# AI-ON/Few-Shot-Music-Generation

Hardware: AMD Instinct MI355X
Metric: episodes/s (LSTM-baseline train step, synthetic vocab=10k seq_len=128 5-way/5-shot h=512) (higher is better)
Workload: dtype f32 (bf16x3-split products, fp32 accumulate)

## Files before the change

### few-shot-music-generation_amd/csrc/api_debug.hip

```cpp
#include "fsmg_model.h"

using namespace fsmg;
using namespace fsmg_host;


extern "C" {

int fsmg_debug_clock_begin(fsmg_handle h, int32_t microseconds) {
    if (!h || microseconds <= 0 || microseconds > 1000000) return FSMG_ERR_INVALID;
    BEGIN_CALL(h, true);
    if (!h->probe) HIPCK(h, hipStreamCreateWithFlags(&h->probe, hipStreamNonBlocking));
    if (!h->d_probe) HIPCK(h, hipMalloc((void**)&h->d_probe, 64));
    HIPCK(h, hipMemsetAsync(h->d_probe, 0, 64, h->probe));
    HIPCK(h, launch_clock_probe(h->probe, (long long)microseconds * 100, h->d_probe));
    return FSMG_OK;
}
int fsmg_debug_clock_end(fsmg_handle h, float* ghz) {
    if (!h || !ghz) return FSMG_ERR_INVALID;
    if (!h->probe || !h->d_probe) return fail(h, FSMG_ERR_STATE, "fsmg_debug_clock_end without fsmg_debug_clock_begin");
    BEGIN_CALL(h, true);
    unsigned long long v[2] = {0, 0};
    HIPCK(h, hipStreamSynchronize(h->probe));
    HIPCK(h, hipMemcpy(v, h->d_probe, sizeof(v), hipMemcpyDeviceToHost));
    *ghz = v[1] ? (float)((double)v[0] / (double)v[1] * 0.1) : 0.0f;
    return FSMG_OK;
}

int fsmg_debug_dims(fsmg_handle h, int32_t dims[5]) {
    if (!h || !dims) return FSMG_ERR_INVALID;
    dims[0] = h->Ep; dims[1] = h->Hp; dims[2] = h->V1p; dims[3] = h->lastB; dims[4] = h->T;
    return FSMG_OK;
}

int fsmg_debug_read(fsmg_handle h, const char* what, float* host, int64_t count) {
    if (!h || !what || !host || count <= 0) return FSMG_ERR_INVALID;
    BEGIN_CALL(h);
    const int64_t B = h->lastB, T = h->T, Hp = h->Hp, G4 = h->G4, rows = T * B;
    const float* src = nullptr; int64_t cap = 0;
    auto layer_of = [&](const char* prefix) -> int {
        const size_t n = std::strlen(prefix);
        if (std::strncmp(what, prefix, n) != 0) return -1;
        const int l = std::atoi(what + n);
        return (l >= 0 && l < h->L && std::strlen(what) > n) ? l : -1;
    };
    int l;
    if (!std::strcmp(what, "aux_tries")) { host[0] = (float)h->aux_tries; return FSMG_OK; }
    if (!std::strcmp(what, "fused_softmax")) { host[0] = h->fused_softmax ? 1.0f : 0.0f; if (count > 1) host[1] = h->fs_call ? 1.0f : 0.0f; return FSMG_OK; }
    if (!std::strcmp(what, "xcd_bx3")) { host[0] = h->xcd_bx3 ? 1.0f : 0.0f; return FSMG_OK; }
    if (!std::strcmp(what, "gemm_kinds")) {
        for (int64_t i = 0; i < count && i < 4; ++i) host[i] = (float)h->gemm_kinds[i];
        return FSMG_OK;
    }
    if (!std::strcmp(what, "xov_selfcheck")) {
        const float v[3] = {(float)h->xov_selfcheck_runs, (float)h->xov_passes, (float)h->xov_selfcheck_every};
        for (int64_t i = 0; i < count && i < 3; ++i) host[i] = v[i];
        return FSMG_OK;
    }
    if (!std::strcmp(what, "xcd_partitioned")) {
        host[0] = h->xov ? 1.0f : 0.0f;
        if (count > 1) { const int b = h->lastB > 0 ? h->lastB : 45, rpx = lstm_xcd16_packed_rows(b, h->Hp); host[1] = (h->xov && rpx > 0) ? (float)xov_first_free(b, h->Hp) : 8.0f; }
        if (count > 2) host[2] = h->xov_last ? 1.0f : 0.0f;
        return FSMG_OK;
    }
    if (!std::strcmp(what, "logits")) { src = h->logits; cap = rows * h->V1p; }
    else if (!std::strcmp(what, "dlogits")) { src = dlogits_buf(h); cap = rows * h->V1p; }
    else if (!std::strcmp(what, "lse")) { src = h->lse; cap = rows; }
    else if (!std::strcmp(what, "ce")) { src = h->ce; cap = rows; }
    else if (!std::strcmp(what, "row_weight")) { src = h->roww; cap = h->last_mask_groups > 0 ? rows : 0; }
    else if (!std::strcmp(what, "n_valid")) {
        if (count > h->last_mask_groups) return fail(h, FSMG_ERR_SIZE, "debug read larger than the buffer");
        std::vector<int> nv((size_t)count);
        HIPCK(h, hipStreamSynchronize(h->stream));
        HIPCK(h, hipMemcpy(nv.data(), h->d_nvalid, sizeof(int) * count, hipMemcpyDeviceToHost));
        for (int64_t i = 0; i < count; ++i) host[i] = (float)nv[(size_t)i];
        return FSMG_OK;
    }
    else if (!std::strcmp(what, "dx")) { src = h->dXemb; cap = rows * h->Ep; }
    else if (!std::strcmp(what, "dh")) { src = h->dH; cap = rows * Hp; }
    else if (!std::strcmp(what, "gnorm")) { src = h->d_gnorm; cap = 1; }
    else if (!std::strcmp(what, "tail")) { src = h->G + h->n_flat; cap = FSMG_GRAD_TAIL; }
    else if ((l = layer_of("gates")) >= 0) { src = h->Z[l]; cap = rows * G4; }
    else if ((l = layer_of("h")) >= 0) { src = h->Hs[l]; cap = (T + 1) * B * Hp; }
    else if ((l = layer_of("c")) >= 0) { src = h->Cs[l]; cap = (T + 1) * B * Hp; }
    else return fail(h, FSMG_ERR_NAME, std::string("unknown debug buffer '") + what + "'");
    if (count > cap) return fail(h, FSMG_ERR_SIZE, "debug read larger than the buffer");
    HIPCK(h, hipStreamSynchronize(h->stream));
    HIPCK(h, hipMemcpy(host, src, sizeof(float) * count, hipMemcpyDeviceToHost));
    return FSMG_OK;
}

int fsmg_debug_step_profile(fsmg_handle h, int32_t which, uint64_t* stamps, int64_t cap, int32_t* n_blocks,
                            int32_t* n_waves) {
    if (!h || !stamps || !n_blocks || !n_waves || h->lastB <= 0 || h->T < 3) return FSMG_ERR_INVALID;
    BEGIN_CALL(h);
    { const int rc_cs = ensure_cs(h); if (rc_cs != FSMG_OK) return rc_cs; }
    const int B = h->lastB, Hp = h->Hp, G4 = h->G4, l = h->L - 1, t = h->T / 2;
    const int nb = which == 0 ? (G4 / 16) * ((B + 15) / 16) : (Hp / 16) * ((B + 15) / 16);
    const int nw = which == 0 ? 4 : 8;
    const int64_t n = (int64_t)nb * nw * 8;
    if (cap < n) return fail(h, FSMG_ERR_SIZE, "stamp buffer too small");
    unsigned long long* d = nullptr;
    HIPCK(h, hipMalloc((void**)&d, sizeof(unsigned long long) * n));
    HIPCK(h, hipMemsetAsync(d, 0, sizeof(unsigned long long) * n, h->stream));
    for (int rep = 0; rep < 3; ++rep) {
        if (which == 0) {
            LstmFwdArgs a{};
            const size_t Bp16 = (size_t)(B + 15) / 16 * 16;
            a.KhF = h->khf + (size_t)(2 * l) * Hp * G4; a.hF_prev = h->HF[l] + (size_t)t * Bp16 * Hp;
// ... 54 lines not shown
```

### few-shot-music-generation_amd/csrc/api_schedule.hip

```cpp
#include "fsmg_model.h"

using namespace fsmg;
using namespace fsmg_host;

namespace fsmg_host {

bool use_ws_gemm(fsmg_model* h, int amode, int bmode, const GemmArgs& g, const Lane& ln) {
    const int mode = h->gemm_ws;
    if (!h->bx3 || mode == 0 || ln.lds_pad != 0 || g.xcd_first != 0) return false;
    if (mode == 2) return true;
    const int64_t tiles = ((g.M + 127) / 128) * (int64_t)((g.N + 127) / 128);
    if (amode == OP_KC && bmode == OP_XC) return g.K >= 384 && g.K <= 640 && tiles >= 512;
    if (amode == OP_XC && bmode == OP_XC) return tiles >= 256 && g.M <= 512;
    return g.K <= 4096;
}

bool use_h_gemm(fsmg_model* h, int amode, int bmode, const GemmArgs& g, const Lane& ln) {
    const int mode = h->gemm_h;
    if (!h->bx3 || mode == 0 || ln.lds_pad != 0 || g.xcd_first != 0) return false;
    if (amode == OP_XC && g.gather != nullptr && g.m_split == 0) return false;
    if (mode == 2) return true;
    const int64_t tiles = ((g.M + 255) / 256) * (int64_t)((g.N + 255) / 256);
    if (amode == OP_KC && bmode == OP_KC) return g.K >= 4096 && tiles >= 32;
    if (amode == OP_XC && bmode == OP_XC) {
// ... 37 lines not shown
        return FSMG_OK;
    }
    if (!deferred && slabs == h->slabs && h->slabs_owner != nullptr) GEMMCK(h->slabs_owner->flush());
    if (!deferred && slabs == h->slabs && h->side_pending) {
        HIPCK(h, hipStreamWaitEvent(h->stream, h->ev_side, 0));
        h->side_pending = false;
    }
    if (deferred && sq != nullptr && g.row_scale != nullptr) return fail(h, FSMG_ERR_STATE, "internal: row-scaled GEMM with squared-norm partials");
    float* C = g.C; float* colsum = g.colsum;
    g.C = slabs; g.c_slab = mn; g.ksplit = S;
    if (colsum) { g.colsum = cslabs; g.colsum_slab = g.N; }
    HIPCK(h, launch_gemm(h, s, amode, bmode, g, ln.lds_pad));
    if (deferred) {
        if (sq != nullptr && g.row_scale != nullptr) return fail(h, FSMG_ERR_STATE, "internal: row-scaled GEMM with squared-norm partials");
        GEMMCK(defer->room(colsum ? 2 : 1));
        GEMMCK(defer->reduce(slabs, mn, S, C, mn, sq, g.row_scale, g.N));
        if (colsum) GEMMCK(defer->reduce(cslabs, g.N, S, colsum, g.N));
        if (sq_done) *sq_done = sq != nullptr;
        return FSMG_OK;
    }
    HIPCK(h, launch_reduce_slabs2(s, slabs, mn, S, C, mn, cslabs, g.N, colsum, colsum ? g.N : 0));
    if (g.row_scale != nullptr) HIPCK(h, launch_scale_rows(s, C, g.row_scale, g.M, g.N));
    return FSMG_OK;
}

int select_xcd_format(fsmg_model* h, int B) {
    if (h->Hp != 1024 || !h->bx3 || h->xcd_bx3_forced || h->khx == nullptr || !(h->persist && h->xcd)) return FSMG_OK;
    const bool want = lstm_xcd_bx3_pays(B, (int)h->Hp) && B <= h->xcd_max_rows;
    if (want == h->xcd_bx3) return FSMG_OK;
    h->xcd_bx3 = want;
    drop_graphs(h);
    return repack_recurrent_weights(h, h->stream);
}

void choose_schedule(fsmg_model* h, int B, bool train) {
    h->ov_call = h->overlap && (h->overlap_forced || !use_xcd(h, B));
    h->xov_call = false;
    h->eager_call = h->eager && !h->ov_call && h->persist &&
                    (use_xcd(h, B) || lstm_fwd_chain_supported(B, h->Hp) || lstm_fwd_chain_rt_supported(B, h->Hp));
    if (train && h->xov && ((h->Hp == 512 && h->L == 1) || h->Hp == 1024) && h->xcd_bx3 && h->bx3 && !h->ov_call && h->aux != nullptr && use_xcd(h, B) &&
        (!h->timing || h->timing_only == "lstm_fwd" || h->timing_only == "lstm_bwd")) {
        const int rpx = lstm_xcd16_packed_rows(B, h->Hp);
        h->xov_call = rpx > 0 && xov_first_free(B, h->Hp) <= (h->Hp == 1024 ? 6 : 5);
        if (h->xov_call) h->eager_call = true;
    }
}
void xov_gate(fsmg_model* h, GemmArgs& g, int B) {
    const int rpx = lstm_xcd16_packed_rows(B, h->Hp);
    g.gate = h->xov_prog; g.gate_expect = lstm_xcd_active_blocks(B, rpx, h->Hp); g.gate_rows = B; g.gate_last = h->T - 1;
    g.gate_err = h->d_err; g.gate_spin = h->chain_spin_limit > 0 ? 200000 : 0; g.gate_every = h->xov_pub;
}
int gemm_restricted(fsmg_model* h, hipStream_t s, int amode, int bmode, GemmArgs g, int first, int* ctl) {
    g.bx3 = 3; g.xcd_first = first; g.work = ctl; g.stop = ctl + 2; g.claim = ctl + 4; g.work_limit = gemm_items(g);
    HIPCK(h, launch_gemm(h, s, amode, bmode, g, 0));
    return FSMG_OK;
}
int gemm_prepare_queue(fsmg_model* h, GemmArgs& g, int split, OpBatch* defer, bool* ok) {
    *ok = false;
    const int S = std::max(1, std::min(std::min(split, MAX_SPLIT), g.K / 256));
    const int64_t mn = (int64_t)g.M * g.N;
    const int64_t need = round_up((int64_t)S * mn, 64) + (g.colsum ? round_up((int64_t)S * g.N, 64) : 0);
    if (S < 2 || defer == nullptr || h->arena == nullptr || g.ldc != g.N || h->arena_off + need > h->arena_cap || g.row_scale != nullptr) return FSMG_OK;
    float* slabs = h->arena + h->arena_off; float* cslabs = slabs + round_up((int64_t)S * mn, 64);
    h->arena_off += need;
    float* C = g.C; float* colsum = g.colsum;
    g.C = slabs; g.c_slab = mn; g.ksplit = S; g.bx3 = 3;
    if (colsum) { g.colsum = cslabs; g.colsum_slab = g.N; }
    if (!xov_fits(g)) { h->arena_off -= need; g.C = C; g.colsum = colsum; g.ksplit = 1; return FSMG_OK; }
    GEMMCK(defer->room(colsum ? 2 : 1));
    GEMMCK(defer->reduce(slabs, mn, S, C, mn));
    if (colsum) GEMMCK(defer->reduce(cslabs, g.N, S, colsum, g.N));
    *ok = true;
    return FSMG_OK;
}
int gemm_cleanup(fsmg_model* h, hipStream_t s, int amode, int bmode, GemmArgs g, int* ctl) {
    g.bx3 = 3; g.xcd_first = -1; g.work = ctl; g.claim = ctl + 4;
    HIPCK(h, launch_gemm(h, s, amode, bmode, g, 0));
    return FSMG_OK;
}

}
```

### few-shot-music-generation_amd/csrc/fsmg_model.h

```cpp
#pragma once
#include <atomic>
#include <hip/hip_runtime.h>
#include <dlfcn.h>

#include <algorithm>
#include <cmath>
#include <cstdlib>
#include <new>
#include <cstdio>
#include <cstring>
#include <functional>
#include <map>
#include <mutex>
#include <string>
#include <vector>

#include "../../include/fsmg.h"
#include "fsmg_kernels.h"

namespace fsmg_host {
using namespace fsmg;
struct OpBatch;

inline int64_t round_up(int64_t x, int64_t m) { return (x + m - 1) / m * m; }
// ... 117 lines not shown
    float* inboxX = nullptr; int64_t inboxx_floats = 0;
    int* d_inbox_dirty = nullptr;
    int* tickets = nullptr;
    static constexpr int TICKET_LAUNCHES = 64;
    int ticket_next = 0;
    int64_t n_timeouts = 0, n_persist_launches = 0, n_xcd_launches = 0, n_step_launches = 0;
    bool khf_dirty = true;
    bool lazy_cs = true;
    bool cs_stale = false;
    float* slabs = nullptr;
    float* arena = nullptr;
    int64_t arena_cap = 0, arena_off = 0;
    bool warned_split = false;
    int* tok_first = nullptr; int* tok_count = nullptr;
    bool tok_table_open = false;
    bool last_bwd_xcd = false;
    bool eager = true, eager_call = false;
    const int* cur_sup = nullptr; const int* cur_qry = nullptr;
    float* colsum_slabs = nullptr;
    float* slabs2 = nullptr;
    float* colsum_slabs2 = nullptr;
    hipStream_t probe = nullptr;
    unsigned long long* d_probe = nullptr;
    hipStream_t aux = nullptr;
    int aux_tries = 0;
    static constexpr int NCHUNK = 16;
    static constexpr int nchunk = 8;
    static constexpr int nchunk_persist = 4;
    static constexpr int aux_blocks_persist = 2;
    static constexpr int aux_blocks_per_cu = 2;
    hipEvent_t ev_chunk[NCHUNK] = {};
    hipEvent_t ev_fork = nullptr, ev_join = nullptr;
    bool merge_dk = true;
    hipEvent_t ev_bucket[2] = {};
    bool overlap = true;
    bool overlap_forced = false;
    bool ov_call = false;
    int bx3 = 1;
    int gemm_h = 1;
    int gemm_ws = 1;
    int max_split = fsmg_host::MAX_SPLIT;
    long long gemm_kinds[4] = {};
    bool xov = false, xov_call = false;
    bool xov_eligible = false;
    bool bucket0_recorded = false;
    static constexpr int xov_dw_split = 4;
    static constexpr int xov_pub = 6;
    int xov_strikes = 0;
    bool xov_last = false;
    int xov_parts = 3;
    int* xov_prog = nullptr;
    static constexpr int XOV_CTL = 8192;
    int* xov_ctl = nullptr;
    int64_t slab_cap = 0;
    std::map<std::string, hipGraphExec_t> graphs;
    struct LaunchCounts { int64_t xcd = 0, persist = 0, step = 0; bool bwd_xcd = false; };
    std::map<std::string, LaunchCounts> graph_counts;
    char* gen = nullptr;
    size_t gen_bytes = 0;
    std::vector<fsmg_dstate_s*> dstates;
    std::vector<fsmg_cache_s*> caches;
    char* cat = nullptr;
    size_t cat_bytes = 0;

    void* comm = nullptr; bool own_comm = false; int world = 1, rank = 0;
    hipStream_t comm_stream = nullptr;
    hipEvent_t ev_comm = nullptr;
    int lastB = 0;
    bool have_grads = false;
    bool upd_split = false;
    bool upd_pending = false;
    hipEvent_t ev_upd_fork = nullptr, ev_upd = nullptr;
    float* d_decided = nullptr;
    fsmg_host::OpBatch* slabs_owner = nullptr;
    int xov_selfcheck_left = 2;
    int xov_selfcheck_every = 1000;
    long long xov_passes = 0, xov_selfcheck_runs = 0;
    bool xov_selfcheck_fault = false;
    long long seen_selfcheck_mismatch = 0;
    bool inplace_dlogits = true;
    bool fused_softmax = true;
    bool fs_call = false;
    float* Hsc = nullptr;
    float* crow = nullptr;
    long long seen_softmax_range = 0;
    bool tail_aside = true;
    bool side_pending = false;
    hipEvent_t ev_side_fork = nullptr, ev_side = nullptr;
    hipEvent_t ev_turn = nullptr, ev_turn_aux = nullptr;
    std::atomic<bool> capturing{false};
    std::string err;
    bool timing = false;
    std::string timing_only;
    std::map<std::string, fsmg_host::TimerClass> timers;
};

namespace fsmg_host {

extern thread_local std::string g_create_error;

inline int fail(fsmg_model* h, int code, const std::string& msg) {
    if (h) h->err = msg; else g_create_error = msg;
    return code;
}

template <class Config>
// ... 288 lines not shown
```

### few-shot-music-generation_amd/csrc/gemm.hip

```cpp
#include "fsmg_kernels.h"
#include "gemm_edge.h"
#include <cstdlib>
#include <algorithm>
#include <type_traits>

namespace fsmg {

typedef float f32x16 __attribute__((ext_vector_type(16)));

namespace {

#ifndef FSMG_GEMM_BK
#define FSMG_GEMM_BK 16
#endif
#ifndef FSMG_GEMM_BM
#define FSMG_GEMM_BM 128
#endif
constexpr int BM = FSMG_GEMM_BM, BN = 128, BK = FSMG_GEMM_BK;
constexpr int NTHREADS = 2 * BM;
constexpr int NWAVES = NTHREADS / 64;
constexpr int KQ = BK / 4;
template <int XW> struct Nld { static constexpr int v = XW * BK / 4 / NTHREADS; };
template <int MODE, int XW> struct TileLd { static constexpr int v = (MODE == OP_KC) ? XW + 1 : XW + 4; };

// ... 597 lines not shown
            }
#pragma unroll
            for (int i = 0; i < 2; ++i) {
                const float4 q = *reinterpret_cast<const float4*>(p[i]);
                v[4 * i] = q.x; v[4 * i + 1] = q.y; v[4 * i + 2] = q.z; v[4 * i + 3] = q.w;
                p[i] += step;
            }
        }
    }
    __device__ __forceinline__ void fetch_partial(int k0, int kend, int tid) {
        const long long adv = use_buf ? (long long)(so >> 2) : 0;
        so += sstep;
        if (MODE == OP_XC) {
            const int kh = tid / XW;
            if (gp != nullptr) {
#pragma unroll
                for (int i = 0; i < 8; ++i) v[i] = (k0 + 8 * kh + i < kend) ? p[0][(long long)gi[i] * ld_] : 0.0f;
                advance_ids();
                return;
            }
            const float* q = use_buf ? src_ + (vo[0] >> 2) + adv : p[0];
#pragma unroll
            for (int i = 0; i < 8; ++i) v[i] = (k0 + 8 * kh + i < kend) ? q[i * ld_] : 0.0f;
            if (!use_buf) p[0] += step;
        } else {
            const int kq = tid & 3;
#pragma unroll
            for (int i = 0; i < 2; ++i) {
                const float* q = use_buf ? src_ + (vo[i] >> 2) + adv : p[i];
#pragma unroll
                for (int e = 0; e < 4; ++e) v[4 * i + e] = (k0 + 4 * kq + e < kend) ? q[e] : 0.0f;
                if (!use_buf) p[i] += step;
            }
        }
    }
    __device__ __forceinline__ void load() {}
    __device__ __forceinline__ float sum8() const { return ((v[0] + v[1]) + (v[2] + v[3])) + ((v[4] + v[5]) + (v[6] + v[7])); }
    __device__ __forceinline__ void commit(unsigned char* tile) const {
        unsigned w[3][4];
        split8(v, w);
#pragma unroll
        for (int pl = 0; pl < 3; ++pl) {
            if (MODE == OP_XC) {
                *reinterpret_cast<uint4*>(tile + pl * PLANE + lds_ofs[0]) = make_uint4(w[pl][0], w[pl][1], w[pl][2], w[pl][3]);
            } else {
                *reinterpret_cast<uint2*>(tile + pl * PLANE + lds_ofs[0]) = make_uint2(w[pl][0], w[pl][1]);
                *reinterpret_cast<uint2*>(tile + pl * PLANE + lds_ofs[1]) = make_uint2(w[pl][2], w[pl][3]);
            }
        }
    }
};

typedef __attribute__((address_space(3))) void* bx_lds_ptr_t;
template <int XT, bool GATHER = false>
struct BxDmaXC {
    static constexpr int KH = XT * 16, PLANE = 2 * KH;
    __amdgpu_buffer_rsrc_t rs;
    unsigned vo[2], so, sstep, ldb;
    unsigned char* raw;
    int rd_ofs, lds_ofs, kvalid;
    float v[8];
    const int* gidx; int gk[2], gend; unsigned xofs, gnext[2];
    __device__ __forceinline__ unsigned grow(int i) { const int k = min(gk[i], gend); gk[i] += 16; return gidx ? (unsigned)gidx[k] : (unsigned)k; }
    __device__ __forceinline__ void init(const float* src, int ld, int X, int x0, const int* gather, int kb, int tid, int = 0, unsigned char* raw_ = nullptr, int kend = 0) {
        const int lane = tid & 63, wave = tid >> 6;
        raw = raw_;
        const int xcol = min(x0 + 32 * wave + 4 * (lane & 7), X - 4), krow = lane >> 3;
        ldb = (unsigned)ld * 4u;
        rs = __builtin_amdgcn_make_buffer_rsrc((void*)src, 0, (int)0xfffffffcu, 0x00020000);
        if constexpr (GATHER) {
            gidx = gather; gend = kend - 1; xofs = (unsigned)xcol * 4u;
#pragma unroll
            for (int i = 0; i < 2; ++i) gk[i] = kb + 8 * i + krow;
#pragma unroll
            for (int i = 0; i < 2; ++i) vo[i] = grow(i) * ldb + xofs;
#pragma unroll
            for (int i = 0; i < 2; ++i) gnext[i] = grow(i);
            so = 0; sstep = 0;
        } else {
#pragma unroll
            for (int i = 0; i < 2; ++i) vo[i] = (unsigned)(kb + 8 * i + krow) * ldb + (unsigned)xcol * 4u;
            so = 0; sstep = 16u * ldb;
        }
        rd_ofs = ((lane >> 5) * 256 + (lane & 31)) * 4;
        lds_ofs = (lane >> 5) * KH + (32 * wave + (lane & 31)) * 16;
        kvalid = 16;
    }
    __device__ __forceinline__ void fetch() {
        const unsigned s0 = __builtin_amdgcn_readfirstlane(so);
        __builtin_amdgcn_raw_ptr_buffer_load_lds(rs, (bx_lds_ptr_t)raw, 16, vo[0], s0, 0, 0);
        __builtin_amdgcn_raw_ptr_buffer_load_lds(rs, (bx_lds_ptr_t)(raw + 1024), 16, vo[1], s0, 0, 0);
        if constexpr (GATHER) {
#pragma unroll
            for (int i = 0; i < 2; ++i) { vo[i] = gnext[i] * ldb + xofs; gnext[i] = grow(i); }
        } else {
            so += sstep;
        }
    }
    __device__ __forceinline__ void fetch_partial(int k0, int kend, int tid) {
        if constexpr (GATHER) {
            fetch();
            kvalid = kend - k0;
            return;
        }
        const int krow = (tid & 63) >> 3;
#pragma unroll
// ... 234 lines not shown
        bx_barrier();
        if (do_colsum && lt < 128 && n0 + lt < g.N) g.colsum[(long long)z * g.colsum_slab + n0 + lt] = csum + s_cs[lt];
    } else {
        const int wm = wave >> 1, wn = wave & 1;
        const int l31 = lane & 31, khalf = lane >> 5;
        f32x16 acc[2][2];
#pragma unroll
        for (int i = 0; i < 2; ++i)
#pragma unroll
            for (int j = 0; j < 2; ++j)
#pragma unroll
                for (int r = 0; r < 16; ++r) acc[i][j][r] = 0.0f;
        const int fa = khalf * (XA * 16) + (wm * 64 + l31) * 16, fb = khalf * 2048 + (wn * 64 + l31) * 16;
        bx_barrier();
        if (PROF) { p_loop = plast = __builtin_amdgcn_s_memtime(); }
        for (int kt = 0; kt < nk; ++kt) {
            const unsigned char* at = smem + (kt & 1) * STAGE;
            const unsigned char* bt = at + A_OPER;
            bf16x8_t a[3][2], b[3][2];
#pragma unroll
            for (int pl = 2; pl >= 0; --pl)
#pragma unroll
                for (int i = 0; i < 2; ++i) {
                    a[pl][i] = *reinterpret_cast<const bf16x8_t*>(at + pl * A_PLANE + fa + i * 512);
                    b[2 - pl][i] = *reinterpret_cast<const bf16x8_t*>(bt + (2 - pl) * BX_PLANE + fb + i * 512);
                }
#define BX_TERM(PA, PB)                                                                                        \
            acc[0][0] = __builtin_amdgcn_mfma_f32_32x32x16_bf16(a[PA][0], b[PB][0], acc[0][0], 0, 0, 0);            \
            acc[0][1] = __builtin_amdgcn_mfma_f32_32x32x16_bf16(a[PA][0], b[PB][1], acc[0][1], 0, 0, 0);            \
            acc[1][0] = __builtin_amdgcn_mfma_f32_32x32x16_bf16(a[PA][1], b[PB][0], acc[1][0], 0, 0, 0);            \
            acc[1][1] = __builtin_amdgcn_mfma_f32_32x32x16_bf16(a[PA][1], b[PB][1], acc[1][1], 0, 0, 0);
            BX_TERM(2, 0) BX_TERM(0, 2) BX_TERM(1, 1) BX_TERM(1, 0) BX_TERM(0, 1) BX_TERM(0, 0)
#undef BX_TERM
            BX_STAMP(2)
            bx_barrier();
            BX_STAMP(4)
        }
        if (PROF) p_exit_loop = __builtin_amdgcn_s_memtime();
        bx_barrier();
        store_tile<EM>(g, acc, reinterpret_cast<float*>(smem), z, m0, n0, tn, tilesN, wave, lane);
    }
    if (PROF && g.prof != nullptr && lane == 0) {
        __builtin_amdgcn_s_waitcnt(0);
        const unsigned long long p_end = __builtin_amdgcn_s_memtime();
        unsigned hw, xcc;
        asm volatile("s_getreg_b32 %0, hwreg(HW_REG_HW_ID)" : "=s"(hw));
        asm volatile("s_getreg_b32 %0, hwreg(HW_REG_XCC_ID)" : "=s"(xcc));
        unsigned long long* o = g.prof + ((size_t)(blockIdx.y * gridDim.x + blockIdx.x) * (NMW + 4) + wave) * 8;
        o[0] = p_entry; o[1] = p_loop; o[2] = pacc[2]; o[3] = pacc[3]; o[4] = pacc[4]; o[5] = p_exit_loop; o[6] = p_end;
        o[7] = ((unsigned long long)xcc << 32) | hw;
    }
}

template <int AMODE, int BMODE, bool PROF = false, int BUFM = 0, bool QUEUE = false, bool AG = false, int EM = EPI_PLAIN>
__global__ __launch_bounds__(512, 1) void k_gemm_bx3h(const GemmArgs g) {
    constexpr int XT = 256;
    constexpr int PLANE = 2 * XT * 16, OPER = 3 * PLANE;
    constexpr int EPI = 8 * 32 * 68 * 4;
    constexpr bool DMA = BUFM >= 3;
    constexpr int A_BYTES = 2 * OPER, PIPE = 4 * OPER;
    static_assert(PIPE >= EPI, "the epilogue's transpose slices live in the pipeline's LDS");
    constexpr int RAW = DMA ? ((AMODE == OP_XC) + (BMODE == OP_XC)) * 8 * 2048 : 0;
    __shared__ __attribute__((aligned(1024))) unsigned char smem[PIPE + RAW];
    __shared__ float s_cs[256];
    const int tid = threadIdx.x;
    const int lane = tid & 63, wave = __builtin_amdgcn_readfirstlane(tid >> 6);
    const bool late = wave >= 4;
    const int l31 = lane & 31, khalf = lane >> 5;
    const int tilesM = (g.M + XT - 1) / XT, tilesN = (g.N + XT - 1) / XT;
    int tm, tn, z;
    if (QUEUE) {
        __shared__ int s_item;
        const int total = tilesM * tilesN * (g.ksplit > 1 ? g.ksplit : 1);
        if (g.xcd_first > 0) {
            int xcc;
            asm volatile("s_getreg_b32 %0, hwreg(HW_REG_XCC_ID)" : "=s"(xcc));
            if ((xcc & 7) < g.xcd_first) {
                if (g.gate == nullptr) return;
                if (tid == 0) s_item = __hip_atomic_load(g.gate + g.gate_last, __ATOMIC_RELAXED, __HIP_MEMORY_SCOPE_AGENT) >= g.gate_expect;
                __syncthreads();
                const int join = s_item;
                __syncthreads();
                if (!join) return;
            }
        }
        if (tid == 0) {
            int item = -1;
            if (g.xcd_first < 0) {
                const int j = atomicAdd(g.work + 1, 1);
                if (j < total && atomicCAS(g.claim + j, 0, 1) == 0) item = j;
            } else if (__hip_atomic_load(g.stop, __ATOMIC_RELAXED, __HIP_MEMORY_SCOPE_SYSTEM) == 0) {
                const int j = atomicAdd(g.work, 1);
                if (j < min(g.work_limit, total) && atomicCAS(g.claim + j, 0, 1) == 0) item = j;
            }
            if (item >= 0 && g.gate != nullptr) {
                const int tm_ = (item / tilesN) % tilesM;
                int t_need = (min(g.M, (tm_ + 1) * XT) - 1) / g.gate_rows;
                if (g.gate_every > 1) t_need = min(g.gate_last, (t_need / g.gate_every + 1) * g.gate_every - 1);
                const int spin_cap = g.gate_spin;
                for (int spins = 0; __hip_atomic_load(g.gate + t_need, __ATOMIC_RELAXED, __HIP_MEMORY_SCOPE_AGENT) < g.gate_expect; ++spins) {
                    __builtin_amdgcn_s_sleep(32);
                    if (spins >= spin_cap || ((spins & 63) == 63 && __hip_atomic_load(g.gate_err, __ATOMIC_RELAXED, __HIP_MEMORY_SCOPE_AGENT) == 2)) {
                        __hip_atomic_store(g.gate_err, 2, __ATOMIC_RELAXED, __HIP_MEMORY_SCOPE_AGENT);
                        item = -1;
                        break;
                    }
                }
            }
            s_item = item;
        }
        __syncthreads();
        const int item = s_item;
        if (item < 0) return;
        tm = (item / tilesN) % tilesM; tn = item % tilesN; z = item / (tilesM * tilesN);
    } else {
        const int bid = xcd_tile(blockIdx.x, tilesM * tilesN);
        tile_coords(bid, tilesM, tilesN, g.group_m, tm, tn);
        z = blockIdx.y;
    }
    const int m0 = tm * XT, n0 = tn * XT;
    const GemmEdgeWave ew = gemm_edge_wave(min(XT, g.M - m0), min(XT, g.N - n0), wave);
    const int wm = __builtin_amdgcn_readfirstlane(ew.wm), wn = __builtin_amdgcn_readfirstlane(ew.wn);
    const bool live = __builtin_amdgcn_readfirstlane((int)ew.live) != 0;
    unsigned long long pacc[5] = {0, 0, 0, 0, 0}, plast = 0, p_entry = 0, p_loop = 0;
    if (PROF) { p_entry = plast = __builtin_amdgcn_s_memtime(); }

    int kb = 0, ke = g.K;
    if (g.ksplit > 1) {
        const int per = ((g.K + g.ksplit - 1) / g.ksplit + 15) / 16 * 16;
        kb = z * per;
        ke = min(g.K, kb + per);
    }
    const int nk = (ke > kb) ? (ke - kb + 15) / 16 : 0;
    const int nfull = (ke > kb) ? (ke - kb) / 16 : 0;

    typename BxStagerSel<DMA, AMODE, XT, 512, (BUFM >= 2), AG>::type sa;
    typename BxStagerSel<DMA, BMODE, XT, 512, (BUFM >= 1)>::type sb;
    if constexpr (AG) {
        static_assert(!AG || (DMA && AMODE == OP_XC), "two-part A: LDS-DMA staged x-contiguous operand");
        const bool first = m0 < g.m_split;
        sa.init(first ? g.A : g.A2, first ? g.lda : g.lda2, first ? g.m_split : g.M - g.m_split, first ? m0 : m0 - g.m_split,
                first ? g.gather : nullptr, kb, tid, g.K, smem + PIPE + wave * 2048, ke);
    } else
    if constexpr (DMA && AMODE == OP_XC) sa.init(g.A, g.lda, g.M, m0, nullptr, kb, tid, g.K, smem + PIPE + wave * 2048);
    else sa.init(g.A, g.lda, g.M, m0, g.gather, kb, tid, g.K);
    if constexpr (DMA && BMODE == OP_XC) sb.init(g.B, g.ldb, g.N, n0, nullptr, kb, tid, g.K, smem + PIPE + ((AMODE == OP_XC) ? 8 * 2048 : 0) + wave * 2048);
    else sb.init(g.B, g.ldb, g.N, n0, nullptr, kb, tid, g.K);

    f32x16 acc[4][2];
#pragma unroll
    for (int i = 0; i < 4; ++i)
#pragma unroll
        for (int j = 0; j < 2; ++j)
#pragma unroll
            for (int r = 0; r < 16; ++r) acc[i][j][r] = 0.0f;

    const bool do_colsum = (BMODE == OP_XC) && g.colsum != nullptr && tm == 0;
    float csum = 0.0f;
    constexpr bool WCS = AMODE == OP_XC && BMODE == OP_XC;
    const bool cs_weighted = WCS && do_colsum && g.colsum_w != nullptr;
    const float* cs_p = (WCS && g.colsum_w != nullptr ? g.colsum_w : g.B) + kb + 8 * ((DMA && BMODE == OP_XC) ? (lane >> 5) : (tid >> 8)) + (lane & 7);
    float cs_wv = 0.0f;
    unsigned char* const smemB = smem + A_BYTES;
#define BXH_FETCH(T)                                                                                           \
    if ((T) < nfull) { sa.fetch(); sb.fetch(); }                                                               \
    else { sa.fetch_partial(kb + (T) * 16, ke, tid); sb.fetch_partial(kb + (T) * 16, ke, tid); }               \
    if constexpr (WCS) cs_wv = cs_p[(T) * 16];
#define BXH_COMMIT(ST)                                                                                         \
    sa.load();                                                                                                 \
    sb.load();                                                                                                 \
    if (do_colsum) {                                                                                           \
        if (cs_weighted) {                \
// ... 15 lines not shown
    const int fa = khalf * (XT * 16) + (wm * 128 + l31) * 16, fb = khalf * (XT * 16) + (wn * 64 + l31) * 16;
    if (PROF) { p_loop = plast = __builtin_amdgcn_s_memtime(); }
    if (!live) {
        for (int kt = 0; kt < nk; ++kt) {
            if (kt + 1 < nk) {
                BXH_COMMIT((kt + 1) & 1)
                if (kt + 2 < nk) { BXH_FETCH(kt + 2) }
            }
            bx_barrier();
        }
    } else
    for (int kt = 0; kt < nk; ++kt) {
        const bool more = kt + 1 < nk;
        constexpr bool READS_ALL_FIRST = AMODE == OP_KC && BMODE == OP_KC;
        const unsigned char* at = smem + (kt & 1) * OPER;
        const unsigned char* bt = smemB + (kt & 1) * OPER;
        bf16x8_t a[3][4], b[3][2];
#define BXH_READ_A(pl) _Pragma("unroll") for (int i = 0; i < 4; ++i) a[pl][i] = *reinterpret_cast<const bf16x8_t*>(at + (pl) * PLANE + fa + i * 512);
#define BXH_READ_B(pl) _Pragma("unroll") for (int j = 0; j < 2; ++j) b[pl][j] = *reinterpret_cast<const bf16x8_t*>(bt + (pl) * PLANE + fb + j * 512);
        BXH_READ_A(2) BXH_READ_B(0)
        if (READS_ALL_FIRST) { BXH_READ_A(0) BXH_READ_B(2) BXH_READ_A(1) BXH_READ_B(1) }
        __builtin_amdgcn_sched_barrier(0);
        if (late && more) {
            BXH_COMMIT((kt + 1) & 1)
            if (kt + 2 < nk) { BXH_FETCH(kt + 2) }
        }
        __builtin_amdgcn_sched_barrier(0);
        BX_STAMP(3)
        if (!READS_ALL_FIRST) { BXH_READ_A(0) BXH_READ_B(2) BXH_READ_A(1) BXH_READ_B(1) }
#undef BXH_READ_A
#undef BXH_READ_B
#define BXH_TERM(PA, PB)                                                                                       \
        _Pragma("unroll") for (int i = 0; i < 4; ++i)                                                          \
        _Pragma("unroll") for (int j = 0; j < 2; ++j)                                                          \
            acc[i][j] = __builtin_amdgcn_mfma_f32_32x32x16_bf16(a[PA][i], b[PB][j], acc[i][j], 0, 0, 0);
        BXH_TERM(2, 0) BXH_TERM(0, 2) BXH_TERM(1, 1) BXH_TERM(1, 0) BXH_TERM(0, 1) BXH_TERM(0, 0)
#undef BXH_TERM
        BX_STAMP(2)
        if (!late && more) {
            BXH_COMMIT((kt + 1) & 1)
            if (kt + 2 < nk) { BXH_FETCH(kt + 2) }
        }
        BX_STAMP(3)
        bx_barrier();
        BX_STAMP(4)
    }
#undef BXH_FETCH
#undef BXH_COMMIT
    const unsigned long long p_exit_loop = PROF ? __builtin_amdgcn_s_memtime() : 0;

    if (do_colsum) {
        const int col = (DMA && BMODE == OP_XC) ? 32 * wave + (lane & 31) : (tid & 255);
        const bool upper = (DMA && BMODE == OP_XC) ? lane >= 32 : tid >= 256;
        if (upper) s_cs[col] = csum;
        bx_barrier();
        if (!upper && n0 + col < g.N) g.colsum[(long long)z * g.colsum_slab + n0 + col] = csum + s_cs[col];
    }
    float* ep = reinterpret_cast<float*>(smem) + wave * (32 * 68);
    if (PROF && (g.dbg & 8)) {
        float sink = 0.0f;
#pragma unroll
        for (int i = 0; i < 4; ++i)
#pragma unroll
            for (int j = 0; j < 2; ++j)
#pragma unroll
                for (int r = 0; r < 16; ++r) sink += acc[i][j][r];
        if (sink == 1.2345e-30f) g.C[0] = sink;
    } else
    if ((n0 + wn * 64) / 128 < (g.N + 127) / 128) {
        const EpiBias bias = epi_bias<EM>(g, z, n0 + wn * 64, lane);
#pragma unroll
        for (int h2 = 0; h2 < 2; ++h2) {
            f32x16 (&sub)[2][2] = *reinterpret_cast<f32x16 (*)[2][2]>(&acc[2 * h2][0]);
            store_tile_at<EM>(g, sub, ep, z, m0 + wm * 128 + h2 * 64, n0 + wn * 64, (n0 + wn * 64) / 128, (g.N + 127) / 128, wn & 1, lane, bias);
        }
    }
    if (PROF && g.prof != nullptr && lane == 0) {
        __builtin_amdgcn_s_waitcnt(0);
        const unsigned long long p_end = __builtin_amdgcn_s_memtime();
        unsigned hw, xcc;
        asm volatile("s_getreg_b32 %0, hwreg(HW_REG_HW_ID)" : "=s"(hw));
        asm volatile("s_getreg_b32 %0, hwreg(HW_REG_XCC_ID)" : "=s"(xcc));
        unsigned long long* o = g.prof + ((size_t)(blockIdx.y * gridDim.x + blockIdx.x) * 8 + wave) * 8;
        o[0] = p_entry; o[1] = p_loop; o[2] = pacc[2]; o[3] = pacc[3]; o[4] = pacc[4]; o[5] = p_exit_loop; o[6] = p_end;
        o[7] = ((unsigned long long)xcc << 32) | hw;
    }
}
#undef BX_STAMP

#define FSMG_LAUNCH_EPI(GRID, BLOCK, LDS, KERNEL, ...)                                                                          \
    do {                                                                                                                        \
        if constexpr (AMODE == OP_KC && BMODE == OP_XC) {                                                                       \
            if (em == EPI_CE_STORE) { hipLaunchKernelGGL((KERNEL<__VA_ARGS__, EPI_CE_STORE>), GRID, BLOCK, LDS, s, g); break; } \
            if (em == EPI_CE_FWD) { hipLaunchKernelGGL((KERNEL<__VA_ARGS__, EPI_CE_FWD>), GRID, BLOCK, LDS, s, g); break; }     \
        }                                                                                                                       \
        hipLaunchKernelGGL((KERNEL<__VA_ARGS__, EPI_PLAIN>), GRID, BLOCK, LDS, s, g);                                           \
    } while (0)

template <int AMODE, int BMODE>
hipError_t launch_t(hipStream_t s, const GemmArgs& g, int lds_pad) {
    const int tilesM = (g.M + BM - 1) / BM, tilesN = (g.N + BN - 1) / BN;
    if (g.colsum_w != nullptr && !(g.bx3 == 3 && AMODE == OP_XC && BMODE == OP_XC && g.colsum != nullptr)) return hipErrorInvalidValue;
    if (g.ce_store && !(g.bx3 != 0 && g.ce_part != nullptr && g.ksplit <= 1)) return hipErrorInvalidValue;
    const int em = g.ce_part == nullptr ? EPI_PLAIN : g.ce_store ? EPI_CE_STORE : EPI_CE_FWD;
    const bool split_kernel = g.bx3 != 0 && (g.xcd_first == 0 || g.bx3 == 3);
    if (split_kernel && em != EPI_PLAIN && !(AMODE == OP_KC && BMODE == OP_XC)) return hipErrorInvalidValue;
    if (g.xcd_first != 0 && g.bx3 == 3) {
        if (g.work == nullptr || g.claim == nullptr || (g.xcd_first > 0 && g.stop == nullptr) || g.gather != nullptr || g.prof != nullptr) return hipErrorInvalidValue;
        const long long a_b = 4LL * g.lda * (AMODE == OP_KC ? g.M : g.K), b_b = 4LL * g.ldb * (BMODE == OP_KC ? g.N : g.K);
        if (a_b >= 0xfffff000LL || b_b >= 0xfffff000LL) return hipErrorInvalidValue;
        const int total = ((g.M + 255) / 256) * ((g.N + 255) / 256) * (g.ksplit > 1 ? g.ksplit : 1);
        const int lim = g.work_limit < total ? g.work_limit : total;
        const int blocks = g.xcd_first > 0 ? (int)(((long long)lim * 8 + 7 - g.xcd_first) / (8 - g.xcd_first)) + 64 : total;
        const bool a_dma = AMODE != OP_XC || (g.lda % 4 == 0 && g.M % 4 == 0 && ((uintptr_t)g.A & 15) == 0);
        const bool b_dma = BMODE != OP_XC || (g.ldb % 4 == 0 && g.N % 4 == 0 && ((uintptr_t)g.B & 15) == 0);
        if constexpr (AMODE == OP_XC && BMODE == OP_XC) {
            if (g.m_split > 0) {
                const bool ok = g.m_split % 256 == 0 && g.m_split < g.M && g.A2 != nullptr && b_dma && g.lda % 4 == 0 && g.lda2 % 4 == 0 &&
                                (g.M - g.m_split) % 4 == 0 && (((uintptr_t)g.A | (uintptr_t)g.A2) & 15) == 0 && 4LL * g.lda2 * g.K < 0xfffff000LL;
                if (!ok) return hipErrorInvalidValue;
                FSMG_LAUNCH_EPI(dim3(blocks), dim3(512), 0, k_gemm_bx3h, AMODE, BMODE, false, 3, true, true);
                return hipGetLastError();
            }
            if (a_dma && b_dma) { FSMG_LAUNCH_EPI(dim3(blocks), dim3(512), 0, k_gemm_bx3h, AMODE, BMODE, false, 3, true, false); return hipGetLastError(); }
        }
        if (g.m_split > 0) return hipErrorInvalidValue;
        FSMG_LAUNCH_EPI(dim3(blocks), dim3(512), 0, k_gemm_bx3h, AMODE, BMODE, false, 2, true, false);
        return hipGetLastError();
    }
    if (g.xcd_first != 0) {
        if (g.work == nullptr || g.claim == nullptr || (g.xcd_first > 0 && g.stop == nullptr) || (AMODE == OP_XC && g.gather != nullptr)) return hipErrorInvalidValue;
        const int total = tilesM * tilesN * (g.ksplit > 1 ? g.ksplit : 1);
        const int lim = g.work_limit < total ? g.work_limit : total;
        const int blocks = g.xcd_first > 0 ? (int)(((long long)lim * 8 + 7 - g.xcd_first) / (8 - g.xcd_first)) + 64 : total;
        hipLaunchKernelGGL((k_gemm_queue<AMODE, BMODE>), dim3(blocks), dim3(NTHREADS), lds_pad, s, g);
        return hipGetLastError();
    }
    dim3 grid(tilesM * tilesN, g.ksplit > 1 ? g.ksplit : 1);
    const long long a_bytes = 4LL * g.lda * (AMODE == OP_KC ? g.M : g.K), b_bytes = 4LL * g.ldb * (BMODE == OP_KC ? g.N : g.K);
    const bool a_buf = g.gather == nullptr && a_bytes < 0xfffff000LL, b_buf = b_bytes < 0xfffff000LL;
    static const bool buf_off = std::getenv("FSMG_GEMM_BUF") && std::atoi(std::getenv("FSMG_GEMM_BUF")) == 0;
    const int bufm = (buf_off && g.prof == nullptr) ? 0 : (a_buf && b_buf) ? 2 : (b_buf ? 1 : 0);
#ifdef FSMG_EXPERIMENTS
    if (g.prof != nullptr && bufm != 2) return hipErrorInvalidValue;
#else
    if (g.prof != nullptr) return hipErrorInvalidValue;
#endif
    if (g.bx3 == 3) {
        dim3 grid3(((g.M + 255) / 256) * ((g.N + 255) / 256), g.ksplit > 1 ? g.ksplit : 1);
        if (g.m_split > 0) {
            if constexpr (AMODE == OP_XC && BMODE == OP_XC) {
                const bool ok = g.m_split % 256 == 0 && g.m_split < g.M && g.A2 != nullptr && g.prof == nullptr && b_buf &&
                                g.lda % 4 == 0 && g.lda2 % 4 == 0 && (g.M - g.m_split) % 4 == 0 && g.ldb % 4 == 0 && g.N % 4 == 0 &&
                                (((uintptr_t)g.A | (uintptr_t)g.A2 | (uintptr_t)g.B) & 15) == 0 && 4LL * g.lda2 * g.K < 0xfffff000LL &&
                                (g.gather != nullptr || 4LL * g.lda * g.K < 0xfffff000LL);
                if (!ok) return hipErrorInvalidValue;
                FSMG_LAUNCH_EPI(grid3, dim3(512), lds_pad, k_gemm_bx3h, AMODE, BMODE, false, 3, false, true);
                return hipGetLastError();
            }
            return hipErrorInvalidValue;
        }
        const bool dma_off = !gemm_dma_enabled();
        const bool a_dma = AMODE != OP_XC || (g.lda % 4 == 0 && g.M % 4 == 0 && ((uintptr_t)g.A & 15) == 0);
        const bool b_dma = BMODE != OP_XC || (g.ldb % 4 == 0 && g.N % 4 == 0 && ((uintptr_t)g.B & 15) == 0);
        const bool dma = !dma_off && bufm == 2 && a_dma && b_dma;
        if constexpr (AMODE == OP_XC && BMODE == OP_XC) {
// ... 106 lines not shown
```

Measured before the change: 625.0.

## Make queued bx3 GEMM blocks persistent, looping over claimed work items

The queued bx3h GEMM kernel now splits the per-tile body into a device function and has each block loop, claiming work items from the atomic queue until it runs dry, instead of one item per block. The launch grid is capped at 256 blocks rather than one block per item. The aim is to cut block launch and scheduling overhead and let fewer resident blocks drain the queue, at the risk of load imbalance and serialization within the capped grid. It also counts first-claimers in a control word and adds a debug read for queue item counts.

```diff
diff --git a/few-shot-music-generation_amd/csrc/api_debug.hip b/few-shot-music-generation_amd/csrc/api_debug.hip
--- a/few-shot-music-generation_amd/csrc/api_debug.hip
+++ b/few-shot-music-generation_amd/csrc/api_debug.hip
@@ -54,6 +54,15 @@
     if (!std::strcmp(what, "xov_selfcheck")) {
         const float v[3] = {(float)h->xov_selfcheck_runs, (float)h->xov_passes, (float)h->xov_selfcheck_every};
         for (int64_t i = 0; i < count && i < 3; ++i) host[i] = v[i];
+        return FSMG_OK;
+    }
+    if (!std::strcmp(what, "xov_walk")) {
+        int drew[2] = {0, 0};
+        if (h->xov_ctl == nullptr) return fail(h, FSMG_ERR_STATE, "no queue words");
+        HIPCK(h, hipStreamSynchronize(h->stream));
+        for (int i = 0; i < 2; ++i) HIPCK(h, hipMemcpy(&drew[i], h->xov_ctl + i * fsmg_model::XOV_CTL + 3, sizeof(int), hipMemcpyDeviceToHost));
+        const float v[4] = {(float)h->xov_queue_items[0], (float)drew[0], (float)h->xov_queue_items[1], (float)drew[1]};
+        for (int64_t i = 0; i < count && i < 4; ++i) host[i] = v[i];
         return FSMG_OK;
     }
     if (!std::strcmp(what, "xcd_partitioned")) {
diff --git a/few-shot-music-generation_amd/csrc/api_schedule.hip b/few-shot-music-generation_amd/csrc/api_schedule.hip
--- a/few-shot-music-generation_amd/csrc/api_schedule.hip
+++ b/few-shot-music-generation_amd/csrc/api_schedule.hip
@@ -113,6 +113,7 @@
 }
 int gemm_restricted(fsmg_model* h, hipStream_t s, int amode, int bmode, GemmArgs g, int first, int* ctl) {
     g.bx3 = 3; g.xcd_first = first; g.work = ctl; g.stop = ctl + 2; g.claim = ctl + 4; g.work_limit = gemm_items(g);
+    h->xov_queue_items[ctl != h->xov_ctl] = g.work_limit;
     HIPCK(h, launch_gemm(h, s, amode, bmode, g, 0));
     return FSMG_OK;
 }
diff --git a/few-shot-music-generation_amd/csrc/fsmg_model.h b/few-shot-music-generation_amd/csrc/fsmg_model.h
--- a/few-shot-music-generation_amd/csrc/fsmg_model.h
+++ b/few-shot-music-generation_amd/csrc/fsmg_model.h
@@ -193,6 +193,7 @@
     int* xov_prog = nullptr;
     static constexpr int XOV_CTL = 8192;
     int* xov_ctl = nullptr;
+    int xov_queue_items[2] = {0, 0};
     int64_t slab_cap = 0;
     std::map<std::string, hipGraphExec_t> graphs;
     struct LaunchCounts { int64_t xcd = 0, persist = 0, step = 0; bool bwd_xcd = false; };
diff --git a/few-shot-music-generation_amd/csrc/gemm.hip b/few-shot-music-generation_amd/csrc/gemm.hip
--- a/few-shot-music-generation_amd/csrc/gemm.hip
+++ b/few-shot-music-generation_amd/csrc/gemm.hip
@@ -673,6 +673,7 @@
 };
 
 typedef __attribute__((address_space(3))) void* bx_lds_ptr_t;
+typedef __attribute__((address_space(3))) int* bx_lds_int_t;
 template <int XT, bool GATHER = false>
 struct BxDmaXC {
     static constexpr int KH = XT * 16, PLANE = 2 * KH;
@@ -1013,8 +1014,8 @@
     }
 }
 
-template <int AMODE, int BMODE, bool PROF = false, int BUFM = 0, bool QUEUE = false, bool AG = false, int EM = EPI_PLAIN>
-__global__ __launch_bounds__(512, 1) void k_gemm_bx3h(const GemmArgs g) {
+template <int AMODE, int BMODE, bool PROF, int BUFM, bool AG, int EM>
+__device__ __forceinline__ void bx3h_tile(const GemmArgs& g, const int tid, const int tilesN, const int tm, const int tn, const int z) {
     constexpr int XT = 256;
     constexpr int PLANE = 2 * XT * 16, OPER = 3 * PLANE;
     constexpr int EPI = 8 * 32 * 68 * 4;
@@ -1024,61 +1025,9 @@
     constexpr int RAW = DMA ? ((AMODE == OP_XC) + (BMODE == OP_XC)) * 8 * 2048 : 0;
     __shared__ __attribute__((aligned(1024))) unsigned char smem[PIPE + RAW];
     __shared__ float s_cs[256];
-    const int tid = threadIdx.x;
     const int lane = tid & 63, wave = __builtin_amdgcn_readfirstlane(tid >> 6);
     const bool late = wave >= 4;
     const int l31 = lane & 31, khalf = lane >> 5;
-    const int tilesM = (g.M + XT - 1) / XT, tilesN = (g.N + XT - 1) / XT;
-    int tm, tn, z;
-    if (QUEUE) {
-        __shared__ int s_item;
-        const int total = tilesM * tilesN * (g.ksplit > 1 ? g.ksplit : 1);
-        if (g.xcd_first > 0) {
-            int xcc;
-            asm volatile("s_getreg_b32 %0, hwreg(HW_REG_XCC_ID)" : "=s"(xcc));
-            if ((xcc & 7) < g.xcd_first) {
-                if (g.gate == nullptr) return;
-                if (tid == 0) s_item = __hip_atomic_load(g.gate + g.gate_last, __ATOMIC_RELAXED, __HIP_MEMORY_SCOPE_AGENT) >= g.gate_expect;
-                __syncthreads();
-                const int join = s_item;
-                __syncthreads();
-                if (!join) return;
-            }
-        }
-        if (tid == 0) {
-            int item = -1;
-            if (g.xcd_first < 0) {
-                const int j = atomicAdd(g.work + 1, 1);
-                if (j < total && atomicCAS(g.claim + j, 0, 1) == 0) item = j;
-            } else if (__hip_atomic_load(g.stop, __ATOMIC_RELAXED, __HIP_MEMORY_SCOPE_SYSTEM) == 0) {
-                const int j = atomicAdd(g.work, 1);
-                if (j < min(g.work_limit, total) && atomicCAS(g.claim + j, 0, 1) == 0) item = j;
-            }
-            if (item >= 0 && g.gate != nullptr) {
-                const int tm_ = (item / tilesN) % tilesM;
-                int t_need = (min(g.M, (tm_ + 1) * XT) - 1) / g.gate_rows;
-                if (g.gate_every > 1) t_need = min(g.gate_last, (t_need / g.gate_every + 1) * g.gate_every - 1);
-                const int spin_cap = g.gate_spin;
-                for (int spins = 0; __hip_atomic_load(g.gate + t_need, __ATOMIC_RELAXED, __HIP_MEMORY_SCOPE_AGENT) < g.gate_expect; ++spins) {
-                    __builtin_amdgcn_s_sleep(32);
-                    if (spins >= spin_cap || ((spins & 63) == 63 && __hip_atomic_load(g.gate_err, __ATOMIC_RELAXED, __HIP_MEMORY_SCOPE_AGENT) == 2)) {
-                        __hip_atomic_store(g.gate_err, 2, __ATOMIC_RELAXED, __HIP_MEMORY_SCOPE_AGENT);
-                        item = -1;
-                        break;
-                    }
-                }
-            }
-            s_item = item;
-        }
-        __syncthreads();
-        const int item = s_item;
-        if (item < 0) return;
-        tm = (item / tilesN) % tilesM; tn = item % tilesN; z = item / (tilesM * tilesN);
-    } else {
-        const int bid = xcd_tile(blockIdx.x, tilesM * tilesN);
-        tile_coords(bid, tilesM, tilesN, g.group_m, tm, tn);
-        z = blockIdx.y;
-    }
     const int m0 = tm * XT, n0 = tn * XT;
     const GemmEdgeWave ew = gemm_edge_wave(min(XT, g.M - m0), min(XT, g.N - n0), wave);
     const int wm = __builtin_amdgcn_readfirstlane(ew.wm), wn = __builtin_amdgcn_readfirstlane(ew.wn);
@@ -1200,9 +1149,11 @@
     if (do_colsum) {
         const int col = (DMA && BMODE == OP_XC) ? 32 * wave + (lane & 31) : (tid & 255);
         const bool upper = (DMA && BMODE == OP_XC) ? lane >= 32 : tid >= 256;
-        if (upper) s_cs[col] = csum;
+        __attribute__((address_space(3))) float* cs = (__attribute__((address_space(3))) float*)s_cs;
+        asm volatile("" : "+v"(cs));
+        if (upper) cs[col] = csum;
         bx_barrier();
-        if (!upper && n0 + col < g.N) g.colsum[(long long)z * g.colsum_slab + n0 + col] = csum + s_cs[col];
+        if (!upper && n0 + col < g.N) g.colsum[(long long)z * g.colsum_slab + n0 + col] = csum + cs[col];
     }
     float* ep = reinterpret_cast<float*>(smem) + wave * (32 * 68);
     if (PROF && (g.dbg & 8)) {
@@ -1235,6 +1186,77 @@
     }
 }
 #undef BX_STAMP
+
+template <int AMODE, int BMODE, bool PROF = false, int BUFM = 0, bool QUEUE = false, bool AG = false, int EM = EPI_PLAIN>
+__global__ __launch_bounds__(512, 1) void k_gemm_bx3h(const GemmArgs g) {
+    constexpr int XT = 256;
+    const int tid = threadIdx.x;
+    const int tilesM = (g.M + XT - 1) / XT, tilesN = (g.N + XT - 1) / XT;
+    if constexpr (!QUEUE) {
+        int tm, tn;
+        const int bid = xcd_tile(blockIdx.x, tilesM * tilesN);
+        tile_coords(bid, tilesM, tilesN, g.group_m, tm, tn);
+        bx3h_tile<AMODE, BMODE, PROF, BUFM, AG, EM>(g, tid, tilesN, tm, tn, blockIdx.y);
+    } else {
+        __shared__ int s_item;
+        const int total = tilesM * tilesN * (g.ksplit > 1 ? g.ksplit : 1);
+        if (g.xcd_first > 0) {
+            int xcc;
+            asm volatile("s_getreg_b32 %0, hwreg(HW_REG_XCC_ID)" : "=s"(xcc));
+            if ((xcc & 7) < g.xcd_first) {
+                if (g.gate == nullptr) return;
+                if (tid == 0) s_item = __hip_atomic_load(g.gate + g.gate_last, __ATOMIC_RELAXED, __HIP_MEMORY_SCOPE_AGENT) >= g.gate_expect;
+                __syncthreads();
+                const int join = s_item;
+                __syncthreads();
+                if (!join) return;
+            }
+        }
+        const int wave0 = __builtin_amdgcn_readfirstlane(tid >> 6);
+        for (bool first = true;; first = false) {
+            int one;
+            bx_lds_int_t item_slot = (bx_lds_int_t)&s_item;
+            asm volatile("v_mov_b32 %0, 1" : "=v"(one));
+            asm volatile("" : "+v"(item_slot));
+            int tid_item;
+            asm volatile("v_mbcnt_lo_u32_b32 %0, -1, 0\n\tv_mbcnt_hi_u32_b32 %0, -1, %0" : "=v"(tid_item));
+            tid_item += wave0 * 64;
+            if (tid_item == 0) {
+                int item = -1;
+                if (g.xcd_first < 0) {
+                    for (int j; item < 0 && (j = atomicAdd(g.work + 1, one)) < total;)
+                        if (atomicCAS(g.claim + j, 0, one) == 0) item = j;
+                } else {
+                    const int lim = min(g.work_limit, total);
+                    for (int j; item < 0 && __hip_atomic_load(g.stop, __ATOMIC_RELAXED, __HIP_MEMORY_SCOPE_SYSTEM) == 0 &&
+                                __hip_atomic_load(g.work + 1, __ATOMIC_RELAXED, __HIP_MEMORY_SCOPE_AGENT) == 0 && (j = atomicAdd(g.work, one)) < lim;)
+                        if (atomicCAS(g.claim + j, 0, one) == 0) item = j;
+                }
+                item = __builtin_amdgcn_readfirstlane(item);
+                if (item >= 0 && first) atomicAdd(g.work + 3, one);
+                if (item >= 0 && g.gate != nullptr) {
+                    const int tm_ = (item / tilesN) % tilesM;
+                    int t_need = (min(g.M, (tm_ + 1) * XT) - 1) / g.gate_rows;
+                    if (g.gate_every > 1) t_need = min(g.gate_last, (t_need / g.gate_every + 1) * g.gate_every - 1);
+                    const int spin_cap = g.gate_spin;
+                    for (int spins = 0; __hip_atomic_load(g.gate + t_need, __ATOMIC_RELAXED, __HIP_MEMORY_SCOPE_AGENT) < g.gate_expect; ++spins) {
+                        __builtin_amdgcn_s_sleep(32);
+                        if (spins >= spin_cap || ((spins & 63) == 63 && __hip_atomic_load(g.gate_err, __ATOMIC_RELAXED, __HIP_MEMORY_SCOPE_AGENT) == 2)) {
+                            __hip_atomic_store(g.gate_err, one + one, __ATOMIC_RELAXED, __HIP_MEMORY_SCOPE_AGENT);
+                            item = -1;
+                            break;
+                        }
+                    }
+                }
+                *item_slot = item;
+            }
+            __syncthreads();
+            const int item = __builtin_amdgcn_readfirstlane(*item_slot);
+            if (item < 0) return;
+            bx3h_tile<AMODE, BMODE, PROF, BUFM, AG, EM>(g, tid_item, tilesN, (item / tilesN) % tilesM, item % tilesN, item / (tilesM * tilesN));
+        }
+    }
+}
 
 #define FSMG_LAUNCH_EPI(GRID, BLOCK, LDS, KERNEL, ...)                                                                          \
     do {                                                                                                                        \
@@ -1259,7 +1281,8 @@
         if (a_b >= 0xfffff000LL || b_b >= 0xfffff000LL) return hipErrorInvalidValue;
         const int total = ((g.M + 255) / 256) * ((g.N + 255) / 256) * (g.ksplit > 1 ? g.ksplit : 1);
         const int lim = g.work_limit < total ? g.work_limit : total;
-        const int blocks = g.xcd_first > 0 ? (int)(((long long)lim * 8 + 7 - g.xcd_first) / (8 - g.xcd_first)) + 64 : total;
+        const int one_each = g.xcd_first > 0 ? (int)(((long long)lim * 8 + 7 - g.xcd_first) / (8 - g.xcd_first)) + 64 : total;
+        const int blocks = one_each < 256 ? one_each : 256;
         const bool a_dma = AMODE != OP_XC || (g.lda % 4 == 0 && g.M % 4 == 0 && ((uintptr_t)g.A & 15) == 0);
         const bool b_dma = BMODE != OP_XC || (g.ldb % 4 == 0 && g.N % 4 == 0 && ((uintptr_t)g.B & 15) == 0);
         if constexpr (AMODE == OP_XC && BMODE == OP_XC) {
```

Result: no change. 630.5, median of 6 (+0.9%).
